# ico-eagleye/OppositeRenderer

Hardware: AMD Instinct MI355X
Metric: Mpaths/s + ms/frame (1080p Sponza PPM) at 1/2/4/8 GPUs; % HBM roofline (higher is better)
Workload: dtype f32

## Files before the change

oppositerenderer_amd/csrc/orx_device.h:

```cpp
#pragma once
#include <hip/hip_runtime.h>
#include <stdint.h>

#include "orx_bvh_nodes.h"
#include "orx_detmath.h"
#include "orx_scene_types.h"

namespace orx {

__host__ __device__ inline bool refract(f3& r, f3 i, f3 n, float ior) {
    f3 nn = n;
    float negNdotV = dot(i, nn);
    float eta;
    if (negNdotV > 0.0f) {
        eta = ior;
        nn = -n;
        negNdotV = -negNdotV;
    } else {
        eta = 1.f / ior;
    }
    const float k = 1.f - eta * eta * (1.f - negNdotV * negNdotV);
    if (k < 0.0f) {
        r = mk1(0.f);
        return false;
    }
    r = normalize(i * eta - nn * (eta * negNdotV + sqrtf(k)));
    return true;
}

constexpr uint32_t PRD_HIT_EMITTER = 1u << 31;
constexpr uint32_t PRD_ERROR = 1u << 30;
constexpr uint32_t PRD_MISS = 1u << 29;
constexpr uint32_t PRD_HIT_SPECULAR = 1u << 28;
constexpr uint32_t PRD_HIT_NON_SPECULAR = 1u << 27;
constexpr uint32_t PRD_PATH_TRACING = 1u << 26;
constexpr float RT_DEFAULT_MAX = 1.e27f;

struct Rng {
    uint32_t v0, v1, v2, v3, v4, d;
};
struct RngPlanes {
    uint32_t* p[6];
};
__device__ __forceinline__ Rng rng_load(const RngPlanes& P, size_t s) {
    return Rng{P.p[0][s], P.p[1][s], P.p[2][s], P.p[3][s], P.p[4][s], P.p[5][s]};
}
__device__ __forceinline__ void rng_store(const RngPlanes& P, size_t s, const Rng& r) {
    P.p[0][s] = r.v0; P.p[1][s] = r.v1; P.p[2][s] = r.v2;
    P.p[3][s] = r.v3; P.p[4][s] = r.v4; P.p[5][s] = r.d;
}
__host__ __device__ __forceinline__ Rng rng_init(uint64_t seed) {
    uint32_t s0 = ((uint32_t)seed) ^ 0xaad26b49u;
    uint32_t s1 = ((uint32_t)(seed >> 32)) ^ 0xf7dcefddu;
    uint32_t t0 = 1099087573u * s0;
    uint32_t t1 = 2591861531u * s1;
    Rng r;
    r.d = 6615241u + t1 + t0;
    r.v0 = 123456789u + t0;
    r.v1 = 362436069u ^ t0;
    r.v2 = 521288629u + t1;
    r.v3 = 88675123u ^ t1;
    r.v4 = 5783321u + t0;
    return r;
}
__host__ __device__ __forceinline__ uint32_t rng_next(Rng& s) {
    uint32_t t = s.v0 ^ (s.v0 >> 2);
    s.v0 = s.v1;
    s.v1 = s.v2;
    s.v2 = s.v3;
    s.v3 = s.v4;
    s.v4 = (s.v4 ^ (s.v4 << 4)) ^ (t ^ (t << 1));
    s.d += 362437u;
    return s.v4 + s.d;
}
__device__ __forceinline__ float rnd(Rng& s) {
    uint32_t x = rng_next(s);
    float u = __builtin_fmaf((float)x, 2.3283064e-10f, 2.3283064e-10f / 2.0f);
    return maxf(u - ORX_FLT_EPSILON, 0.0f);
}

__device__ __forceinline__ void create_coordinate_system(f3 N, f3& U, f3& V) {
    if (fabsf(N.x) > fabsf(N.y)) {
        float invLength = 1.f / sqrtf(N.x * N.x + N.z * N.z);
        U = mk(-N.z * invLength, 0.f, N.x * invLength);
    } else {
        float invLength = 1.f / sqrtf(N.y * N.y + N.z * N.z);
        U = mk(0.f, N.z * invLength, -N.y * invLength);
    }
    V = cross(N, U);
}
__device__ __forceinline__ f3 sample_hemisphere_cos(f3 normal, float sx, float sy) {
    float theta = orx_acosf(sqrtf(sx));
    float phi = 2.0f * ORX_PI_F * sy;
    float st = orx_sinf(theta);
    float xs = st * orx_cosf(phi);
    float ys = orx_cosf(theta);
    float zs = st * orx_sinf(phi);
    f3 U, V;
    create_coordinate_system(normal, U, V);
    return normalize(U * xs + normal * ys + V * zs);
}
__device__ __forceinline__ f3 sample_hemisphere(f3 normal, float sx, float sy) {
    f3 U, V;
    create_coordinate_system(normal, U, V);
    float phi = 2.0f * ORX_PI_F * sx;
    float r = sqrtf(sy);
    float x = r * orx_cosf(phi);
    float y = r * orx_sinf(phi);
    float z = 1.0f - x * x - y * y;
    z = z > 0.0f ? sqrtf(z) : 0.0f;
    return normalize(U * x + V * y + normal * z);
}
__device__ __forceinline__ f3 sample_unit_sphere(float sx, float sy) {
    f3 v;
    v.z = 1.f - 2.f * sx;
    float phi = 2 * ORX_PI_F * sy;
    float r = sqrtf(1.f - v.z * v.z);
    v.x = r * orx_cosf(phi);
    v.y = r * orx_sinf(phi);
    return v;
}
__device__ __forceinline__ f3 sample_disc(float sx, float sy, f3 center, float radius, f3 normal) {
    f3 U, V;
    create_coordinate_system(normal, U, V);
    float r = sqrtf(sx);
    float theta = 2.f * ORX_PI_F * sy;
    float x = r * orx_cosf(theta);
    float y = r * orx_sinf(theta);
    return center + (U * x + V * y) * radius;
}

struct DevScene {
    uint32_t nq, ns, nt;
    const DevQuad* quads;
    const uint32_t* qmat;
    const DevSphere* spheres;
    const uint32_t* smat;
    const float4* tri_v;
    const float4* tri_n;
    const float2* tri_uv;
    const float4* tri_t;
    const float4* tri_bt;
    const DevTexture* tex;
    uint32_t ntex;
    const uint32_t* tmat;
    const DevMaterial* mats;
    const DevLight* lights;
    uint32_t nl;
    float bs_cx, bs_cy, bs_cz, bs_r;
    const DevNode4* bvh4;
    uint32_t bvh_nodes;
    uint32_t stack_entries;
    float dir_zero;
    unsigned long long* trav_stats;
};

#define ORX_STACK_DECL extern __shared__ uint32_t orx_stack_lds[]
#define ORX_STACK_PTR (&orx_stack_lds[threadIdx.x & 63])
#define ORX_STACK_BYTES(S) ((size_t)((S).stack_entries + 2) * 64 * 4)

struct Hit {
    float t;
    int32_t prim;
    uint32_t slot;
    float b, g;
    f3 sn;
};

__device__ __forceinline__ bool isect_quad(const DevQuad& q, f3 o, f3 d, float tmin, float tmax, float& tout) {
    f3 n = mk(q.nx, q.ny, q.nz);
    float dt = dot(d, n);
    float t = (q.d - dot(n, o)) / dt;
    if (t > tmin && t < tmax) {
        f3 p = o + d * t;
        f3 vi = p - mk(q.ax, q.ay, q.az);
        float a1 = dot(mk(q.v1x, q.v1y, q.v1z), vi);
        if (a1 >= 0 && a1 <= 1) {
            float a2 = dot(mk(q.v2x, q.v2y, q.v2z), vi);
            if (a2 >= 0 && a2 <= 1) {
                tout = t;
                return true;
            }
        }
    }
    return false;
}
__device__ __forceinline__ bool isect_sphere(const DevSphere& s, f3 o, f3 d, float tmin, float tmax, float& tout,
                                             f3& nout) {
    f3 O = o - mk(s.cx, s.cy, s.cz);
    float b = dot(O, d);
    float c = dot(O, O) - s.r * s.r;
    float disc = b * b - c;
    if (disc > 0.0f) {
        float sdisc = sqrtf(disc);
        float root1 = (-b - sdisc);
        if (root1 > tmin && root1 < tmax) {
            tout = root1;
            nout = (O + d * root1) / s.r;
            return true;
        }
        float root2 = (-b + sdisc);
        if (root2 > tmin && root2 < tmax) {
            tout = root2;
            nout = (O + d * root2) / s.r;
            return true;
        }
    }
    return false;
}
__device__ __forceinline__ bool isect_tri(f3 p0, f3 p1, f3 p2, f3 o, f3 d, float tmin, float tmax, float& tout,
                                          float& bout, float& gout) {
    f3 e0 = p1 - p0;
    f3 e1 = p0 - p2;
    f3 n = cross(e1, e0);
    f3 e2 = (p0 - o) * (1.0f / dot(n, d));
    f3 i = cross(d, e2);
    float beta = dot(i, e1);
    float gamma = dot(i, e0);
    float t = dot(n, e2);
    if ((t < tmax) & (t > tmin) & (beta >= 0.0f) & (gamma >= 0.0f) & (beta + gamma <= 1)) {
        tout = t;
        bout = beta;
        gout = gamma;
        return true;
    }
    return false;
}
__device__ __forceinline__ f3 ld_f3(const float4& v) { return mk(v.x, v.y, v.z); }

struct RayBox {
    f3 o, inv;
    bool nx, ny, nz;
    f3 oinv;
};
__device__ __forceinline__ RayBox ray_box(f3 o, f3 d, float zero = 1e-30f) {
    auto safe = [zero](float v) { return fabsf(v) > zero ? v : copysignf(zero, v); };
    RayBox rb;
    rb.o = o;
    rb.inv = mk(__builtin_amdgcn_rcpf(safe(d.x)), __builtin_amdgcn_rcpf(safe(d.y)), __builtin_amdgcn_rcpf(safe(d.z)));
    rb.nx = rb.inv.x < 0.f;
    rb.ny = rb.inv.y < 0.f;
    rb.nz = rb.inv.z < 0.f;
    rb.oinv = mk(-o.x * rb.inv.x, -o.y * rb.inv.y, -o.z * rb.inv.z);
    return rb;
}
constexpr float ORX_BOX_TMIN = 1.f - 0x1p-20f, ORX_BOX_TMAX = 1.f + 0x1p-20f;
__device__ __forceinline__ void node_test_q(const float4 A, const float4 B, const float4 C, const float4 D,
                                            const RayBox& rb, float tmin, float tmax, float t[4], uint32_t c[4]) {
    const float sx = A.w, sy = D.z, sz = D.w;
    const float ax = (A.x - rb.o.x) * rb.inv.x, bx = sx * rb.inv.x;
    const float ay = (A.y - rb.o.y) * rb.inv.y, by = sy * rb.inv.y;
    const float az = (A.z - rb.o.z) * rb.inv.z, bz = sz * rb.inv.z;
    const uint32_t lx = __float_as_uint(B.x), ly = __float_as_uint(B.y), lz = __float_as_uint(B.z);
    const uint32_t hx = __float_as_uint(B.w), hy = __float_as_uint(C.x), hz = __float_as_uint(C.y);
    const uint32_t nxq = rb.nx ? hx : lx, fxq = rb.nx ? lx : hx;
    const uint32_t nyq = rb.ny ? hy : ly, fyq = rb.ny ? ly : hy;
    const uint32_t nzq = rb.nz ? hz : lz, fzq = rb.nz ? lz : hz;
    c[0] = __float_as_uint(C.z);
    c[1] = __float_as_uint(C.w);
    c[2] = __float_as_uint(D.x);
    c[3] = __float_as_uint(D.y);
    typedef float v2q __attribute__((ext_vector_type(2)));
    auto q2 = [](uint32_t w, int i) {
        return v2q{(float)((w >> (8 * i)) & 0xffu), (float)((w >> (8 * i + 8)) & 0xffu)};
    };
    const v2q ax2 = v2q{ax, ax}, bx2 = v2q{bx, bx}, ay2 = v2q{ay, ay}, by2 = v2q{by, by};
    const v2q az2 = v2q{az, az}, bz2 = v2q{bz, bz};
#pragma unroll
    for (int h = 0; h < 2; h++) {
        const v2q tnx = __builtin_elementwise_fma(q2(nxq, 2 * h), bx2, ax2);
        const v2q tfx = __builtin_elementwise_fma(q2(fxq, 2 * h), bx2, ax2);
        const v2q tny = __builtin_elementwise_fma(q2(nyq, 2 * h), by2, ay2);
        const v2q tfy = __builtin_elementwise_fma(q2(fyq, 2 * h), by2, ay2);
        const v2q tnz = __builtin_elementwise_fma(q2(nzq, 2 * h), bz2, az2);
        const v2q tfz = __builtin_elementwise_fma(q2(fzq, 2 * h), bz2, az2);
#pragma unroll
        for (int e = 0; e < 2; e++) {
            const int i = 2 * h + e;
            const float t0 = fmaxf(fmaxf(fmaxf(tnx[e], tny[e]), tnz[e]), tmin);
            const float t1 = fminf(fminf(fminf(tfx[e], tfy[e]), tfz[e]), tmax);
            t[i] = t0 <= t1 ? t0 : INFINITY;
        }
    }
}
__device__ __forceinline__ __amdgpu_buffer_rsrc_t orx_rsrc(const void* p) {
    return __builtin_amdgcn_make_buffer_rsrc(const_cast<void*>(p), 0, 0xffffffff, 0x00020000);
}
__device__ __forceinline__ float4 ld16(__amdgpu_buffer_rsrc_t r, uint32_t bo) {
    typedef uint32_t u4b __attribute__((ext_vector_type(4)));
    const u4b v = __builtin_amdgcn_raw_buffer_load_b128(r, (int)bo, 0, 0);
    return make_float4(__uint_as_float(v.x), __uint_as_float(v.y), __uint_as_float(v.z), __uint_as_float(v.w));
}
__device__ __forceinline__ void node_test(const DevBvh4* nodes, uint32_t idx, const RayBox& rb, float tmin, float tmax,
                                          float t[4], uint32_t c[4]) {
    const __amdgpu_buffer_rsrc_t r = orx_rsrc(nodes);
    const uint32_t bo = idx << 6;
    node_test_q(ld16(r, bo), ld16(r, bo + 16), ld16(r, bo + 32), ld16(r, bo + 48), rb, tmin, tmax, t, c);
}
typedef float v2t __attribute__((ext_vector_type(2)));
__device__ __forceinline__ void node_test(const DevBvh4F* nodes, uint32_t idx, const RayBox& rb, float tmin, float tmax,
                                          float t[4], uint32_t c[4]) {
    const float* base = reinterpret_cast<const float*>(nodes + idx);
    const float4 NX = *(const float4*)(base + (rb.nx ? 4 : 0)), FX = *(const float4*)(base + (rb.nx ? 0 : 4));
    const float4 NY = *(const float4*)(base + (rb.ny ? 12 : 8)), FY = *(const float4*)(base + (rb.ny ? 8 : 12));
    const float4 NZ = *(const float4*)(base + (rb.nz ? 20 : 16)), FZ = *(const float4*)(base + (rb.nz ? 16 : 20));
    const uint4 CC = *(const uint4*)(base + 24);
    c[0] = CC.x;
    c[1] = CC.y;
    c[2] = CC.z;
    c[3] = CC.w;
    const v2t ix = v2t{rb.inv.x, rb.inv.x}, iy = v2t{rb.inv.y, rb.inv.y}, iz = v2t{rb.inv.z, rb.inv.z};
    const v2t ox = v2t{rb.oinv.x, rb.oinv.x}, oy = v2t{rb.oinv.y, rb.oinv.y}, oz = v2t{rb.oinv.z, rb.oinv.z};
    const v2t tnx0 = __builtin_elementwise_fma(v2t{NX.x, NX.y}, ix, ox), tnx1 = __builtin_elementwise_fma(v2t{NX.z, NX.w}, ix, ox);
    const v2t tfx0 = __builtin_elementwise_fma(v2t{FX.x, FX.y}, ix, ox), tfx1 = __builtin_elementwise_fma(v2t{FX.z, FX.w}, ix, ox);
    const v2t tny0 = __builtin_elementwise_fma(v2t{NY.x, NY.y}, iy, oy), tny1 = __builtin_elementwise_fma(v2t{NY.z, NY.w}, iy, oy);
    const v2t tfy0 = __builtin_elementwise_fma(v2t{FY.x, FY.y}, iy, oy), tfy1 = __builtin_elementwise_fma(v2t{FY.z, FY.w}, iy, oy);
    const v2t tnz0 = __builtin_elementwise_fma(v2t{NZ.x, NZ.y}, iz, oz), tnz1 = __builtin_elementwise_fma(v2t{NZ.z, NZ.w}, iz, oz);
    const v2t tfz0 = __builtin_elementwise_fma(v2t{FZ.x, FZ.y}, iz, oz), tfz1 = __builtin_elementwise_fma(v2t{FZ.z, FZ.w}, iz, oz);
    const float tn[4][3] = {{tnx0.x, tny0.x, tnz0.x}, {tnx0.y, tny0.y, tnz0.y}, {tnx1.x, tny1.x, tnz1.x}, {tnx1.y, tny1.y, tnz1.y}};
    const float tf[4][3] = {{tfx0.x, tfy0.x, tfz0.x}, {tfx0.y, tfy0.y, tfz0.y}, {tfx1.x, tfy1.x, tfz1.x}, {tfx1.y, tfy1.y, tfz1.y}};
#pragma unroll
    for (int i = 0; i < 4; i++) {
        const float t0 = fmaxf(fmaxf(fmaxf(tn[i][0], tn[i][1]), tn[i][2]), tmin);
        const float t1 = fminf(fminf(fminf(tf[i][0], tf[i][1]), tf[i][2]), tmax);
        t[i] = (t0 <= t1 && c[i] != 0xffffffffu) ? t0 : INFINITY;
    }
}
__device__ __forceinline__ void cswap(float& ta, uint32_t& ca, float& tb, uint32_t& cb) {
    const uint32_t ua = __float_as_uint(ta), ub = __float_as_uint(tb);
    const bool sw = ub < ua;
    const uint32_t c = sw ? cb : ca;
    cb = sw ? ca : cb;
    ca = c;
    ta = __uint_as_float(ua < ub ? ua : ub);
    tb = __uint_as_float(ua < ub ? ub : ua);
}

struct StackL {
    uint32_t* s;
    __device__ __forceinline__ void push(int& sp, uint32_t v) const { s[(sp++) * 64] = v; }
    __device__ __forceinline__ uint32_t pop(int& sp) const { return s[(--sp) * 64]; }
    __device__ __forceinline__ void put(int k, uint32_t v) const { s[k * 64] = v; }
    __device__ __forceinline__ bool shallow(int, int) const { return true; }
    __device__ __forceinline__ void put_l(int k, uint32_t v) const { put(k, v); }
    __device__ __forceinline__ uint32_t pop_l(int& sp) const { return pop(sp); }
};
template <int NL>
struct StackH {
    uint32_t* s;
    __amdgpu_buffer_rsrc_t g;
    uint32_t lane;
    static constexpr uint32_t gstride = 64;
    static constexpr size_t lds_bytes() { return (size_t)(NL + 1) * 64 * 4; }
    __host__ __device__ static constexpr uint32_t deep(uint32_t entries) { return entries + 2 > NL ? entries + 2 - NL : 1u; }
    __device__ __forceinline__ StackH(uint32_t* s_, uint32_t* g_, uint32_t blk, uint32_t ndeep, uint32_t lane_)
        : s(s_), g(__builtin_amdgcn_make_buffer_rsrc(g_ + (size_t)blk * ndeep * 64u, 0, ndeep * 256u, 0x00020000)),
          lane(lane_) {}
    __device__ __forceinline__ void push(int& sp, uint32_t v) const { put(sp++, v); }
    __device__ __forceinline__ uint32_t pop(int& sp) const {
        --sp;
        uint32_t v = s[(sp < NL ? sp : NL) * 64];
        if (sp >= NL) v = __builtin_amdgcn_raw_buffer_load_b32(g, (int)(((uint32_t)(sp - NL) * gstride + lane) * 4u), 0, 0);
        return v;
    }
    __device__ __forceinline__ void put(int k, uint32_t v) const {
        s[(k < NL ? k : NL) * 64] = v;
        if (k >= NL) __builtin_amdgcn_raw_buffer_store_b32(v, g, (int)(((uint32_t)(k - NL) * gstride + lane) * 4u), 0, 0);
    }
    __device__ __forceinline__ bool shallow(int sp, int n) const { return !__ballot(sp + n > NL); }
    __device__ __forceinline__ void put_l(int k, uint32_t v) const { s[k * 64] = v; }
    __device__ __forceinline__ uint32_t pop_l(int& sp) const { return s[(--sp) * 64]; }
};
struct NodesG {
    __device__ __forceinline__ void test(const DevScene& S, uint32_t idx, const RayBox& rb, float tmin, float tmax,
                                         float t[4], uint32_t c[4]) const {
        node_test(S.bvh4, idx, rb, tmin, tmax, t, c);
    }
};

#ifdef ORX_TRAV_STATS
#define ORX_TS_DECL uint32_t ts_nodes = 0, ts_leaves = 0, ts_tris = 0, ts_wn = 0, ts_wl = 0
#define ORX_TS_INC(v, n) (v) += (n)
#define ORX_TS_WAVE(v) (v) += ((uint32_t)(__ffsll((unsigned long long)__ballot(1)) - 1) == (threadIdx.x & 63u))
#define ORX_TS_DECL_TOP uint32_t ts_top[4] = {0, 0, 0, 0}
#define ORX_TS_TOP(idx)                                                     \
    do {                                                                    \
        ts_top[0] += (idx) < 21u;                                           \
        ts_top[1] += (idx) < 85u;                                           \
        ts_top[2] += (idx) < 341u;                                          \
        ts_top[3] += (idx) < 1365u;                                         \
    } while (0)
#define ORX_TS_FLUSH_TOP()                                                  \
    do {                                                                    \
        for (int q_ = 0; q_ < 4; q_++) atomicAdd(&S.trav_stats[16 + q_], (unsigned long long)ts_top[q_]); \
    } while (0)
#define ORX_TS_FLUSH(base)                                                  \
    do {                                                                    \
        atomicAdd(&S.trav_stats[(base) + 0], 1ull);                       \
        atomicAdd(&S.trav_stats[(base) + 1], (unsigned long long)ts_nodes);  \
        atomicAdd(&S.trav_stats[(base) + 2], (unsigned long long)ts_leaves); \
        atomicAdd(&S.trav_stats[(base) + 3], (unsigned long long)ts_tris);   \
        atomicAdd(&S.trav_stats[8 + (base) / 2], (unsigned long long)ts_wn);  \
        atomicAdd(&S.trav_stats[9 + (base) / 2], (unsigned long long)ts_wl);  \
    } while (0)
#else
#define ORX_TS_DECL
#define ORX_TS_DECL_TOP
#define ORX_TS_TOP(idx)
#define ORX_TS_FLUSH_TOP()
#define ORX_TS_INC(v, n)
#define ORX_TS_WAVE(v)
#define ORX_TS_FLUSH(base)
#endif

template <class STK, class NODES>
__device__ inline bool trace_closest_t(const DevScene& S, f3 o, f3 d, float tmin, float tmax, Hit& h, const STK& stk,
                                       const NODES& nodes) {
    float best = tmax;
    int32_t bp = -1;
    uint32_t bslot = 0;
    float t;
    for (uint32_t i = 0; i < S.nq; i++) {
        if (isect_quad(S.quads[i], o, d, tmin, best, t)) {
            best = t;
            bp = (int32_t)i;
        }
    }
    f3 sn = mk1(0);
    for (uint32_t i = 0; i < S.ns; i++) {
        f3 n;
        if (isect_sphere(S.spheres[i], o, d, tmin, best, t, n)) {
            best = t;
            bp = (int32_t)(S.nq + i);
            sn = n;
        }
    }
    float bb = 0, bg = 0;
    if (S.nt) {
        const uint32_t base = S.nq + S.ns;
        const RayBox rb = ray_box(o, d, S.dir_zero);
        const float tmin_box = tmin * ORX_BOX_TMIN;
        int sp = 0;
        uint32_t ref = 0;
        ORX_TS_DECL;
        ORX_TS_DECL_TOP;
        uint32_t lf = 0;
        while (ref != ORX_DONE) {
            while (!(ref & ORX_LEAF) && ref != ORX_DONE) {
                float ct[4];
                uint32_t cc[4];
                nodes.test(S, ref, rb, tmin_box, best * ORX_BOX_TMAX, ct, cc);
                ORX_TS_INC(ts_nodes, 1);
                ORX_TS_TOP(ref);
                ORX_TS_WAVE(ts_wn);
                cswap(ct[0], cc[0], ct[1], cc[1]);
                cswap(ct[2], cc[2], ct[3], cc[3]);
                cswap(ct[0], cc[0], ct[2], cc[2]);
                cswap(ct[1], cc[1], ct[3], cc[3]);
                cswap(ct[1], cc[1], ct[2], cc[2]);
                {
                    const int n3 = ct[3] != INFINITY, n2 = ct[2] != INFINITY, n1 = ct[1] != INFINITY;
                    if (stk.shallow(sp, 3)) {
                        stk.put_l(sp, cc[3]);
                        stk.put_l(sp + n3, cc[2]);
                        stk.put_l(sp + n3 + n2, cc[1]);
                        sp += n3 + n2 + n1;
                        ref = ct[0] != INFINITY ? cc[0] : (sp ? stk.pop_l(sp) : ORX_DONE);
                    } else {
                        stk.put(sp, cc[3]);
                        stk.put(sp + n3, cc[2]);
                        stk.put(sp + n3 + n2, cc[1]);
                        sp += n3 + n2 + n1;
                        ref = ct[0] != INFINITY ? cc[0] : (sp ? stk.pop(sp) : ORX_DONE);
                    }
                }
                if ((ref & ORX_LEAF) && !(lf & ORX_LEAF)) {
                    lf = ref;
                    ref = sp ? stk.pop(sp) : ORX_DONE;
                }
                if (!__ballot(!(lf & ORX_LEAF))) break;
            }
            while (lf & ORX_LEAF) {
                const uint32_t first = (lf & 0x7fffffffu) >> 3, cnt = (lf & 7u) + 1u;
                ORX_TS_INC(ts_leaves, 1);
                ORX_TS_INC(ts_tris, cnt);
                ORX_TS_WAVE(ts_wl);
                const __amdgpu_buffer_rsrc_t tr = orx_rsrc(S.tri_v);
                for (uint32_t k = first; k < first + cnt; k++) {
                    const uint32_t tb = k * 48u;
                    const float4 v0 = ld16(tr, tb), v1 = ld16(tr, tb + 16), v2 = ld16(tr, tb + 32);
                    const int32_t gid = (int32_t)(base + __float_as_uint(v0.w));
                    float b, g;
                    float lim = bp >= 0 ? orx_as_float(orx_as_uint(best) + 1u) : best;
                    if (isect_tri(ld_f3(v0), ld_f3(v1), ld_f3(v2), o, d, tmin, lim, t, b, g) &&
                        (t < best || gid < bp)) {
                        best = t;
                        bp = gid;
                        bslot = k;
                        bb = b;
                        bg = g;
                    }
                }
                lf = ref;
                if (ref & ORX_LEAF) ref = sp ? stk.pop(sp) : ORX_DONE;
            }
        }
        ORX_TS_FLUSH(0);
        ORX_TS_FLUSH_TOP();
    }
    if (bp < 0) return false;
    h.t = best;
    h.prim = bp;
    h.slot = bslot;
    h.b = bb;
    h.g = bg;
    h.sn = sn;
    return true;
}
__device__ __forceinline__ bool trace_closest(const DevScene& S, f3 o, f3 d, float tmin, float tmax, Hit& h,
                                              uint32_t* stk) {
    return trace_closest_t(S, o, d, tmin, tmax, h, StackL{stk}, NodesG{});
}

template <class STK, class NODES>
__device__ inline bool trace_any_t(const DevScene& S, f3 o, f3 d, float tmin, float tmax, const STK& stk,
                                   const NODES& nodes) {
    float t;
    for (uint32_t i = 0; i < S.nq; i++)
        if (isect_quad(S.quads[i], o, d, tmin, tmax, t)) return true;
    for (uint32_t i = 0; i < S.ns; i++) {
        f3 n;
        if (isect_sphere(S.spheres[i], o, d, tmin, tmax, t, n)) return true;
    }
    if (S.nt) {
        const RayBox rb = ray_box(o, d, S.dir_zero);
        const float tmin_box = tmin * ORX_BOX_TMIN, tmax_box = tmax * ORX_BOX_TMAX;
        int sp = 0;
        uint32_t ref = 0;
        ORX_TS_DECL;
        uint32_t lf = 0;
        while (ref != ORX_DONE) {
            while (!(ref & ORX_LEAF) && ref != ORX_DONE) {
                float ct[4];
                uint32_t cc[4];
                nodes.test(S, ref, rb, tmin_box, tmax_box, ct, cc);
                ORX_TS_INC(ts_nodes, 1);
                ORX_TS_WAVE(ts_wn);
                const int h0 = ct[0] != INFINITY, h1 = ct[1] != INFINITY, h2 = ct[2] != INFINITY,
                          h3 = ct[3] != INFINITY;
                const uint32_t next = h3 ? cc[3] : h2 ? cc[2] : h1 ? cc[1] : h0 ? cc[0] : ORX_DONE;
                if (stk.shallow(sp, 4)) {
                    stk.put_l(sp, cc[0]);
                    sp += h0;
                    stk.put_l(sp, cc[1]);
                    sp += h1;
                    stk.put_l(sp, cc[2]);
                    sp += h2;
                    stk.put_l(sp, cc[3]);
                    sp += h3;
                    sp -= next != ORX_DONE;
                    ref = next != ORX_DONE ? next : (sp ? stk.pop_l(sp) : ORX_DONE);
                } else {
                    stk.put(sp, cc[0]);
                    sp += h0;
                    stk.put(sp, cc[1]);
                    sp += h1;
                    stk.put(sp, cc[2]);
                    sp += h2;
                    stk.put(sp, cc[3]);
                    sp += h3;
                    sp -= next != ORX_DONE;
                    ref = next != ORX_DONE ? next : (sp ? stk.pop(sp) : ORX_DONE);
                }
                if ((ref & ORX_LEAF) && !(lf & ORX_LEAF)) {
                    lf = ref;
                    ref = sp ? stk.pop(sp) : ORX_DONE;
                }
                if (!__ballot(!(lf & ORX_LEAF))) break;
            }
            while (lf & ORX_LEAF) {
                const uint32_t first = (lf & 0x7fffffffu) >> 3, cnt = (lf & 7u) + 1u;
                ORX_TS_INC(ts_leaves, 1);
                ORX_TS_WAVE(ts_wl);
                const __amdgpu_buffer_rsrc_t tr = orx_rsrc(S.tri_v);
                for (uint32_t k = first; k < first + cnt; k++) {
                    float b, g;
                    ORX_TS_INC(ts_tris, 1);
                    const uint32_t tb = k * 48u;
                    if (isect_tri(ld_f3(ld16(tr, tb)), ld_f3(ld16(tr, tb + 16)), ld_f3(ld16(tr, tb + 32)), o, d,
                                  tmin, tmax, t, b, g)) {
                        ORX_TS_FLUSH(4);
                        return true;
                    }
                }
                lf = ref;
                if (ref & ORX_LEAF) ref = sp ? stk.pop(sp) : ORX_DONE;
            }
        }
        ORX_TS_FLUSH(4);
    }
    return false;
}

__device__ __forceinline__ bool trace_any(const DevScene& S, f3 o, f3 d, float tmin, float tmax, uint32_t* stk) {
    return trace_any_t(S, o, d, tmin, tmax, StackL{stk}, NodesG{});
}

template <class RAYS, class STK>
__device__ __forceinline__ void trace_any_chain_t(const DevScene& S, RAYS& R, const STK& stk) {
    f3 o = mk1(0.f), d = mk1(0.f);
    float tmin = 0.f, tmax = 0.f, tmin_box = 0.f, tmax_box = 0.f;
    RayBox rb = ray_box(o, mk1(1.f), S.dir_zero);
    int sp = 0;
    uint32_t ref = ORX_DONE, lf = 0;
    auto fetch = [&]() -> bool {
        while (R.next(o, d, tmin, tmax)) {
            float t;
            bool hit = false;
            for (uint32_t i = 0; i < S.nq && !hit; i++) hit = isect_quad(S.quads[i], o, d, tmin, tmax, t);
            for (uint32_t i = 0; i < S.ns && !hit; i++) {
                f3 n;
                hit = isect_sphere(S.spheres[i], o, d, tmin, tmax, t, n);
            }
            if (hit || !S.nt) {
                R.result(hit);
                continue;
            }
            rb = ray_box(o, d, S.dir_zero);
            tmin_box = tmin * ORX_BOX_TMIN, tmax_box = tmax * ORX_BOX_TMAX;
            sp = 0;
            ref = 0;
            lf = 0;
            return true;
        }
        return false;
    };
    bool have = fetch();
    const __amdgpu_buffer_rsrc_t tr = orx_rsrc(S.tri_v);
    while (__ballot(have)) {
        if (!have) continue;
        while (!(ref & ORX_LEAF) && ref != ORX_DONE) {
            float ct[4];
            uint32_t cc[4];
            node_test(S.bvh4, ref, rb, tmin_box, tmax_box, ct, cc);
            const int h0 = ct[0] != INFINITY, h1 = ct[1] != INFINITY, h2 = ct[2] != INFINITY, h3 = ct[3] != INFINITY;
            const uint32_t next = h3 ? cc[3] : h2 ? cc[2] : h1 ? cc[1] : h0 ? cc[0] : ORX_DONE;
            if (stk.shallow(sp, 4)) {
                stk.put_l(sp, cc[0]);
                sp += h0;
                stk.put_l(sp, cc[1]);
                sp += h1;
                stk.put_l(sp, cc[2]);
                sp += h2;
                stk.put_l(sp, cc[3]);
                sp += h3;
                sp -= next != ORX_DONE;
                ref = next != ORX_DONE ? next : (sp ? stk.pop_l(sp) : ORX_DONE);
// ... 527 lines not shown
```

oppositerenderer_amd/csrc/orx_kernels.hip:

```cpp
#include <algorithm>
#include <cstdlib>

#include "orx_kernels.h"

namespace orx {

__device__ __forceinline__ uint32_t f2ord(float f) {
    uint32_t u = __float_as_uint(f);
    return (u & 0x80000000u) ? ~u : (u | 0x80000000u);
}
__device__ __forceinline__ float ord2f(uint32_t u) {
    return __uint_as_float((u & 0x80000000u) ? (u & 0x7fffffffu) : ~u);
}
__device__ __forceinline__ float wave_min(float v) {
    for (int o = 32; o > 0; o >>= 1) v = fminf(v, __shfl_xor(v, o, 64));
    return v;
}
__device__ __forceinline__ float wave_max(float v) {
    for (int o = 32; o > 0; o >>= 1) v = fmaxf(v, __shfl_xor(v, o, 64));
    return v;
}
__device__ __forceinline__ uint64_t wave_sum_u64(uint64_t v) {
    for (int o = 32; o > 0; o >>= 1) v += __shfl_xor(v, o, 64);
    return v;
// ... 163 lines not shown
            M.probe = true;
            M.pdepth = P.depth;
            P.o = hitPoint;
            P.tmin = 0.001f;
            M.tmax = st;
            M.inmed = true;
        }
    } else {
        if (MEDIA) M.tmax = RT_DEFAULT_MAX;
        const DevMaterial& m = S.mats[prim_material(S, h)];
        const f3 hitPoint = P.o + P.d * h.t;
        if (m.type == MAT_DIFFUSE || m.type == MAT_GLOSSY || m.type == MAT_TEXTURE) {
            const bool tex = m.type == MAT_TEXTURE;
            const f3 N = shading_normal(S, h);
            if (P.depth >= 1 && P.numStored < pb.D) {
                const uint32_t si = P.p_local * pb.D + P.numStored;
                float4* rec = pb.slots + 4 * (size_t)si;
                rec[0] = make_float4(hitPoint.x, hitPoint.y, hitPoint.z, P.power.x);
                pb.pos4[si] = make_float4(hitPoint.x, hitPoint.y, hitPoint.z, 0.f);
                rec[1] = make_float4(P.d.x, P.d.y, P.d.z, P.power.y);
                rec[2].x = P.power.z;
                if (fmax3(P.power) > 0 || pb.hash) {
                    P.mask |= 1u << P.numStored;
                    lo_x = fminf(lo_x, hitPoint.x); lo_y = fminf(lo_y, hitPoint.y); lo_z = fminf(lo_z, hitPoint.z);
                    hi_x = fmaxf(hi_x, hitPoint.x); hi_y = fmaxf(hi_y, hitPoint.y); hi_z = fmaxf(hi_z, hitPoint.z);
                }
                P.numStored++;
            }
            const f3 Kd = tex ? tex_color(S, m, h) : m.Kd;
            P.power = P.power * Kd;
            P.weight *= fmax3(Kd);
            if (P.depth >= 3) {
                float probContinue = favgf(Kd);
                float probSample = rnd(rs);
                if (probSample >= probContinue) done = true;
                else P.power = P.power / probContinue;
            }
            if (!done) {
                P.depth++;
                if (P.depth >= c.max_photon_depth || (double)P.weight < (tex ? 0.01 : 0.001) ||
                    P.numStored >= pb.Dlim) {
                    done = true;
                } else {
                    float s0 = rnd(rs);
                    float s1 = rnd(rs);
                    P.d = sample_hemisphere_cos(N, s0, s1);
                    P.o = hitPoint;
                    P.tmin = tex ? 0.01f : 0.0001f;
                    if (MEDIA) M.inmed = false;
                }
            }
        } else if (m.type == MAT_EMITTER) {
            if (MEDIA && !M.inmed) P.depth++;
            done = true;
        } else if (m.type == MAT_MIRROR) {
            const f3 N = shading_normal(S, h);
            P.depth++;
            if (P.depth <= c.max_photon_depth) {
                P.power = P.power * m.Kr;
                P.d = reflect(P.d, N);
                P.o = hitPoint;
                P.tmin = 0.0001f;
                if (MEDIA) M.inmed = false;
            } else {
                done = true;
            }
        } else {
            const f3 wsn = shading_normal(S, h);
            const bool outside = dot(wsn, P.d) < 0;
            const f3 N = outside ? wsn : -wsn;
            const float n1 = outside ? 1.0f : m.ior, n2 = outside ? m.ior : 1.0f;
            f3 refr;
            bool valid;
            const float refl = glass_reflect_factor(P.d, N, n1, n2, refr, valid);
            const float sample = rnd(rs);
            const bool reflected = sample <= refl;
            const f3 nd = reflected ? reflect(P.d, N) : refr;
            P.depth++;
            if (P.depth <= c.max_photon_depth) {
                P.o = hitPoint;
                P.d = nd;
                P.tmin = 0.0001f;
                if (MEDIA) M.inmed = (outside && !reflected) || (!outside && reflected);
            } else {
                done = true;
            }
        }
    }
    if (MEDIA && had_probe && P.depth == M.pdepth) {
        done = true;
        if (rnd(rs) < vm.sig_s / (vm.sig_a + vm.sig_s)) {
            M.nev++;
            M.ev_pos = M.spos;
            M.ev_pow = P.power;
            if (P.depth < c.max_photon_depth) {
                const float s0 = rnd(rs), s1 = rnd(rs);
                P.d = sample_unit_sphere(s0, s1);
                P.o = M.spos;
                P.tmin = 0.001f;
                M.tmax = RT_DEFAULT_MAX;
                M.inmed = false;
                done = false;
            }
        }
    }
    if (done) {
        pb.vmask[P.p_local] = (uint8_t)P.mask;
        rng_store(px.rng, P.slot, rs);
        if (MEDIA) {
            mb.ev_a[P.p_local] = make_float4(M.ev_pos.x, M.ev_pos.y, M.ev_pos.z, __uint_as_float(M.nev));
            mb.ev_b[P.p_local] = make_float4(M.ev_pow.x, M.ev_pow.y, M.ev_pow.z, 0.f);
        }
        return false;
    }
    return true;
}

template <bool MEDIA, class STK, class NODES>
__device__ __forceinline__ bool photon_bounce(const DevScene& S, const PixelBufs& px, const PhotonBufs& pb,
                                              const Consts& c, PhotonPath& P, Rng& rs, const STK& stk,
                                              const NODES& nodes, float& lo_x, float& lo_y, float& lo_z,
                                              float& hi_x, float& hi_y, float& hi_z, const VolMap& vm,
                                              PhotonMedia& M, const MediaBufs& mb) {
    Hit h;
    bool had_probe = false;
    bool hit;
    if (MEDIA) {
        had_probe = M.probe;
        M.probe = false;
        hit = trace_closest_m(S, vm, P.o, P.d, P.tmin, M.tmax, M.inmed, h, stk, nodes);
    } else {
        hit = trace_closest_t(S, P.o, P.d, P.tmin, RT_DEFAULT_MAX, h, stk, nodes);
    }
    return photon_after_hit<MEDIA>(S, px, pb, c, P, rs, hit, h, had_probe, lo_x, lo_y, lo_z, hi_x, hi_y, hi_z, vm, M, mb);
}

__device__ __forceinline__ void photon_bbox_flush(const PhotonBufs& pb, float lo_x, float lo_y, float lo_z, float hi_x,
                                                  float hi_y, float hi_z, uint32_t rep, uint32_t lane) {
    lo_x = wave_min(lo_x); lo_y = wave_min(lo_y); lo_z = wave_min(lo_z);
    hi_x = wave_max(hi_x); hi_y = wave_max(hi_y); hi_z = wave_max(hi_z);
    if (lane < 6) {
        float v = lane == 0 ? lo_x : lane == 1 ? lo_y : lane == 2 ? lo_z : lane == 3 ? hi_x : lane == 4 ? hi_y : hi_z;
        if (lane < 3) {
            if (v != INFINITY) atomicMin(&pb.bbox[lane * BBOX_REPLICAS + rep], f2ord(v));
        } else {
            if (v != -INFINITY) atomicMax(&pb.bbox[lane * BBOX_REPLICAS + rep], f2ord(v));
        }
    }
}

#ifndef ORX_PHOTON_WAVES
#define ORX_PHOTON_WAVES 6
#endif
constexpr int PHOTON_LDS_STACK = 16;
template <bool MEDIA>
__global__ __launch_bounds__(64, ORX_PHOTON_WAVES) void k_ppm_photon(DevScene S, PixelBufs px, PhotonBufs pb, Consts c,
                                                                     MediaBufs mb) {
    ORX_STACK_DECL;
    const uint32_t lane = threadIdx.x;
    const uint32_t total = pb.prows * pb.PW;
    const uint32_t p = blockIdx.x * 64u + lane;
    const StackH<PHOTON_LDS_STACK> stk{ORX_STACK_PTR, pb.tstk, blockIdx.x, pb.tdeep, lane};
    float lo_x = INFINITY, lo_y = INFINITY, lo_z = INFINITY;
    float hi_x = -INFINITY, hi_y = -INFINITY, hi_z = -INFINITY;
    PhotonPath P;
    PhotonMedia M;
    M.tmax = RT_DEFAULT_MAX;
    M.inmed = M.probe = false;
    M.pdepth = M.nev = 0;
    M.spos = M.ev_pos = M.ev_pow = mk1(0.f);
    Rng rs;
    bool alive = p < total;
    if (alive) photon_emit(S, px, pb, p, P, rs);
    while (__ballot(alive)) {
        if (alive)
            alive = photon_bounce<MEDIA>(S, px, pb, c, P, rs, stk, NodesG{}, lo_x, lo_y, lo_z, hi_x, hi_y, hi_z, mb.vm,
                                         M, mb);
    }
    photon_bbox_flush(pb, lo_x, lo_y, lo_z, hi_x, hi_y, hi_z, blockIdx.x & (BBOX_REPLICAS - 1), lane);
}

uint32_t photon_stack_deep(uint32_t entries) { return StackH<PHOTON_LDS_STACK>::deep(entries); }
bool launch_ppm_photon(hipStream_t s, const DevScene& S, const PixelBufs& px, const PhotonBufs& pb, const Consts& c,
                       const MediaBufs* mb) {
    const uint32_t total = pb.prows * pb.PW;
    if (total == 0) return true;
    const uint32_t blocks = (total + 63) / 64;
    if ((size_t)blocks * 64 > pb.tlanes || pb.tdeep < StackH<PHOTON_LDS_STACK>::deep(S.stack_entries)) return false;
    const size_t lds = StackH<PHOTON_LDS_STACK>::lds_bytes();
    if (mb)
        hipLaunchKernelGGL((k_ppm_photon<true>), dim3(blocks), dim3(64), lds, s, S, px, pb, c, *mb);
    else
        hipLaunchKernelGGL((k_ppm_photon<false>), dim3(blocks), dim3(64), lds, s, S, px, pb, c, MediaBufs{});
    return true;
}

__global__ void k_grid_setup(PhotonBufs pb, GridBox gb) {
    __shared__ uint32_t red[6];
    const uint32_t lane = threadIdx.x;
    for (int k = 0; k < 6; k++) {
        uint32_t v = pb.bbox[k * BBOX_REPLICAS + lane];
        for (int o = 32; o > 0; o >>= 1) {
            uint32_t w = (uint32_t)__shfl_xor((int)v, o, 64);
            v = k < 3 ? min(v, w) : max(v, w);
        }
        if (lane == 0) red[k] = v;
        pb.bbox[k * BBOX_REPLICAS + lane] = k < 3 ? 0xffffffffu : 0u;
    }
    __syncthreads();
    if (lane != 0) return;
    uint32_t b[6];
    GridParams* g = pb.grid;
    const bool own = red[0] != 0xffffffffu;
    for (int k = 0; k < 3; k++) {
        g->clo[k] = own ? ord2f(red[k]) : INFINITY;
        g->chi[k] = own ? ord2f(red[k + 3]) : -INFINITY;
    }
    for (int k = 0; k < 6; k++) b[k] = gb.on ? gb.b[k] : red[k];
    bool any = b[0] != 0xffffffffu;
    f3 lo, hi;
    if (any) {
        lo = mk(ord2f(b[0]), ord2f(b[1]), ord2f(b[2]));
        hi = mk(ord2f(b[3]), ord2f(b[4]), ord2f(b[5]));
    } else {
        lo = mk1(0.f);
        hi = mk1(0.f);
    }
    lo = mk(lo.x - 0.0000001f, lo.y - 0.0000001f, lo.z - 0.0000001f);
    hi = mk(hi.x + 0.0000001f, hi.y + 0.0000001f, hi.z + 0.0000001f);
    f3 ext = hi - lo;
    float sceneVolume = ext.x * ext.y * ext.z;
    float minVolumePerCell = sceneVolume / (float)pb.gcells;
    float radiusC = orx_powf(minVolumePerCell, 1.0f / 3.0f);
    f3 ncf = ext / radiusC;
    uint32_t nx = orx_f2u_sat(orx_floorf(ncf.x)), ny = orx_f2u_sat(orx_floorf(ncf.y)),
             nz = orx_f2u_sat(orx_floorf(ncf.z));
    f3 each = mk(ext.x / (float)nx, ext.y / (float)ny, ext.z / (float)nz);
    float smallest = fmax3(each);
    float cellSize = (float)((double)smallest + 0.001);
    f3 f = ext / cellSize;
    uint32_t gx = orx_f2u_sat(orx_ceilf(f.x)), gy = orx_f2u_sat(orx_ceilf(f.y)), gz = orx_f2u_sat(orx_ceilf(f.z));
    gx = gx < 1 ? 1 : gx;
    gy = gy < 1 ? 1 : gy;
    gz = gz < 1 ? 1 : gz;
    uint64_t G = (uint64_t)gx * gy * gz;
    g->ox = lo.x; g->oy = lo.y; g->oz = lo.z;
    g->cell = cellSize;
    g->gx = gx; g->gy = gy; g->gz = gz;
    g->any_valid = any;
    g->photons_visited = 0;
    g->cells_visited = 0;
    if (G > pb.gmax) {
        g->error = 1;
        g->G = 0;
    } else {
        g->error = 0;
        g->G = (uint32_t)G;
    }
}
void launch_grid_setup(hipStream_t s, const PhotonBufs& pb, const GridBox& gb) {
    hipLaunchKernelGGL(k_grid_setup, dim3(1), dim3(64), 0, s, pb, gb);
}

constexpr int SCAN_BLOCK = 1024;

__device__ __forceinline__ uint32_t block_exclusive_scan_256(uint32_t v, uint32_t* total) {
    __shared__ uint32_t ws[4];
    const int lane = threadIdx.x & 63, w = threadIdx.x >> 6;
    uint32_t x = v;
    for (int o = 1; o < 64; o <<= 1) {
        uint32_t y = __shfl_up(x, o, 64);
        if (lane >= o) x += y;
    }
    if (lane == 63) ws[w] = x;
    __syncthreads();
    uint32_t pre = 0;
    for (int q = 0; q < w; q++) pre += ws[q];
    *total = ws[0] + ws[1] + ws[2] + ws[3];
    __syncthreads();
    return pre + x - v;
}

constexpr int32_t DIRQ_BAND = 232;
__device__ __forceinline__ uint32_t dir_q8(float x, float y, float z) {
    if (!(fabsf(x) + fabsf(y) + fabsf(z) <= 1.7325f) || !(fmaxf(fabsf(x), fmaxf(fabsf(y), fabsf(z))) <= 1.0f))
        return 0u;
    const int32_t qx = (int32_t)rintf(x * 127.f), qy = (int32_t)rintf(y * 127.f), qz = (int32_t)rintf(z * 127.f);
    return ((uint32_t)qx & 0xffu) | (((uint32_t)qy & 0xffu) << 8) | (((uint32_t)qz & 0xffu) << 16);
}

__device__ __forceinline__ void grid_put(const PhotonBufs& pb, uint32_t dst, const float4 a, const float4 b, float cz) {
    const size_t P = pb.splane;
    float* o = pb.sorted + dst;
    o[SP_X * P] = a.x;
    o[SP_Y * P] = a.y;
    o[SP_Z * P] = a.z;
    o[SP_DIRQ * P] = __uint_as_float(dir_q8(b.x, b.y, b.z));
    o[SP_DX * P] = b.x;
    o[SP_DY * P] = b.y;
    o[SP_DZ * P] = b.z;
    o[SP_PX * P] = a.w;
    o[SP_PY * P] = b.w;
    o[SP_PZ * P] = cz;
}
__global__ __launch_bounds__(256) void k_grid_permute(PhotonBufs pb) {
    const uint32_t valid = pb.grid->valid;
    const uint32_t T = gridDim.x * blockDim.x;
// ... 1420 lines not shown
```

Before: 1101.

## Use LDS byte-address stack pointer with sentinel and branchless push offsets

Rewrites the BVH traversal stack in trace_closest to track a raw LDS byte address instead of an integer index. An ORX_DONE sentinel sits at the stack base so pops need no empty check. Push offsets come from boolean hit masks instead of comparisons against INFINITY. A separate deep path handles spilling to the global buffer, and the LDS stack grows by one entry to hold the sentinel. The aim is fewer address computations and branches per node visit, at the cost of more code and slightly more LDS per wave, which could reduce occupancy.

```diff
diff --git a/oppositerenderer_amd/csrc/orx_device.h b/oppositerenderer_amd/csrc/orx_device.h
--- a/oppositerenderer_amd/csrc/orx_device.h
+++ b/oppositerenderer_amd/csrc/orx_device.h
@@ -157,7 +157,12 @@
 
 #define ORX_STACK_DECL extern __shared__ uint32_t orx_stack_lds[]
 #define ORX_STACK_PTR (&orx_stack_lds[threadIdx.x & 63])
-#define ORX_STACK_BYTES(S) ((size_t)((S).stack_entries + 2) * 64 * 4)
+#define ORX_STACK_BYTES(S) ((size_t)((S).stack_entries + 3) * 64 * 4)
+typedef __attribute__((address_space(3))) uint32_t orx_lds_u32;
+constexpr uint32_t ORX_STK_STRIDE = 64 * 4;
+__device__ __forceinline__ uint32_t orx_lds_addr(uint32_t* p) { return (uint32_t)(uintptr_t)(orx_lds_u32*)p; }
+__device__ __forceinline__ void orx_lds_st(uint32_t a, uint32_t v) { *(orx_lds_u32*)(uintptr_t)a = v; }
+__device__ __forceinline__ uint32_t orx_lds_ld(uint32_t a) { return *(orx_lds_u32*)(uintptr_t)a; }
 
 struct Hit {
     float t;
@@ -246,7 +251,8 @@
 }
 constexpr float ORX_BOX_TMIN = 1.f - 0x1p-20f, ORX_BOX_TMAX = 1.f + 0x1p-20f;
 __device__ __forceinline__ void node_test_q(const float4 A, const float4 B, const float4 C, const float4 D,
-                                            const RayBox& rb, float tmin, float tmax, float t[4], uint32_t c[4]) {
+                                            const RayBox& rb, float tmin, float tmax, float t[4], uint32_t c[4],
+                                            bool* hit = nullptr, const float miss = INFINITY) {
     const float sx = A.w, sy = D.z, sz = D.w;
     const float ax = (A.x - rb.o.x) * rb.inv.x, bx = sx * rb.inv.x;
     const float ay = (A.y - rb.o.y) * rb.inv.y, by = sy * rb.inv.y;
@@ -279,7 +285,8 @@
             const int i = 2 * h + e;
             const float t0 = fmaxf(fmaxf(fmaxf(tnx[e], tny[e]), tnz[e]), tmin);
             const float t1 = fminf(fminf(fminf(tfx[e], tfy[e]), tfz[e]), tmax);
-            t[i] = t0 <= t1 ? t0 : INFINITY;
+            t[i] = t0 <= t1 ? t0 : miss;
+            if (hit) hit[i] = t0 <= t1;
         }
     }
 }
@@ -292,14 +299,14 @@
     return make_float4(__uint_as_float(v.x), __uint_as_float(v.y), __uint_as_float(v.z), __uint_as_float(v.w));
 }
 __device__ __forceinline__ void node_test(const DevBvh4* nodes, uint32_t idx, const RayBox& rb, float tmin, float tmax,
-                                          float t[4], uint32_t c[4]) {
+                                          float t[4], uint32_t c[4], bool* hit = nullptr, const float miss = INFINITY) {
     const __amdgpu_buffer_rsrc_t r = orx_rsrc(nodes);
     const uint32_t bo = idx << 6;
-    node_test_q(ld16(r, bo), ld16(r, bo + 16), ld16(r, bo + 32), ld16(r, bo + 48), rb, tmin, tmax, t, c);
+    node_test_q(ld16(r, bo), ld16(r, bo + 16), ld16(r, bo + 32), ld16(r, bo + 48), rb, tmin, tmax, t, c, hit, miss);
 }
 typedef float v2t __attribute__((ext_vector_type(2)));
 __device__ __forceinline__ void node_test(const DevBvh4F* nodes, uint32_t idx, const RayBox& rb, float tmin, float tmax,
-                                          float t[4], uint32_t c[4]) {
+                                          float t[4], uint32_t c[4], bool* hit = nullptr, const float miss = INFINITY) {
     const float* base = reinterpret_cast<const float*>(nodes + idx);
     const float4 NX = *(const float4*)(base + (rb.nx ? 4 : 0)), FX = *(const float4*)(base + (rb.nx ? 0 : 4));
     const float4 NY = *(const float4*)(base + (rb.ny ? 12 : 8)), FY = *(const float4*)(base + (rb.ny ? 8 : 12));
@@ -323,7 +330,9 @@
     for (int i = 0; i < 4; i++) {
         const float t0 = fmaxf(fmaxf(fmaxf(tn[i][0], tn[i][1]), tn[i][2]), tmin);
         const float t1 = fminf(fminf(fminf(tf[i][0], tf[i][1]), tf[i][2]), tmax);
-        t[i] = (t0 <= t1 && c[i] != 0xffffffffu) ? t0 : INFINITY;
+        const bool hi = t0 <= t1 && c[i] != 0xffffffffu;
+        t[i] = hi ? t0 : miss;
+        if (hit) hit[i] = hi;
     }
 }
 __device__ __forceinline__ void cswap(float& ta, uint32_t& ca, float& tb, uint32_t& cb) {
@@ -344,6 +353,14 @@
     __device__ __forceinline__ bool shallow(int, int) const { return true; }
     __device__ __forceinline__ void put_l(int k, uint32_t v) const { put(k, v); }
     __device__ __forceinline__ uint32_t pop_l(int& sp) const { return pop(sp); }
+    __device__ __forceinline__ uint32_t addr0() const { return orx_lds_addr(s); }
+    __device__ __forceinline__ bool shallow_a(uint32_t, int, bool) const { return true; }
+    __device__ __forceinline__ void put_a(uint32_t a, uint32_t off, uint32_t v) const { orx_lds_st(a + off, v); }
+    __device__ __forceinline__ uint32_t pop_a(uint32_t& a) const {
+        const uint32_t v = orx_lds_ld(a);
+        a -= ORX_STK_STRIDE;
+        return v;
+    }
 };
 template <int NL>
 struct StackH {
@@ -352,7 +369,7 @@
     uint32_t lane;
     static constexpr uint32_t gstride = 64;
     static constexpr size_t lds_bytes() { return (size_t)(NL + 1) * 64 * 4; }
-    __host__ __device__ static constexpr uint32_t deep(uint32_t entries) { return entries + 2 > NL ? entries + 2 - NL : 1u; }
+    __host__ __device__ static constexpr uint32_t deep(uint32_t entries) { return entries + 3 > NL ? entries + 3 - NL : 1u; }
     __device__ __forceinline__ StackH(uint32_t* s_, uint32_t* g_, uint32_t blk, uint32_t ndeep, uint32_t lane_)
         : s(s_), g(__builtin_amdgcn_make_buffer_rsrc(g_ + (size_t)blk * ndeep * 64u, 0, ndeep * 256u, 0x00020000)),
           lane(lane_) {}
@@ -370,11 +387,27 @@
     __device__ __forceinline__ bool shallow(int sp, int n) const { return !__ballot(sp + n > NL); }
     __device__ __forceinline__ void put_l(int k, uint32_t v) const { s[k * 64] = v; }
     __device__ __forceinline__ uint32_t pop_l(int& sp) const { return s[(--sp) * 64]; }
+    __device__ __forceinline__ uint32_t addr0() const { return orx_lds_addr(s); }
+    __device__ __forceinline__ uint32_t lim() const { return orx_lds_addr(s - lane) + (uint32_t)NL * ORX_STK_STRIDE; }
+    __device__ __forceinline__ bool shallow_a(uint32_t a, int n, bool need) const {
+        return !__ballot(need && a >= lim() - (uint32_t)n * ORX_STK_STRIDE);
+    }
+    __device__ __forceinline__ void put_a(uint32_t a, uint32_t off, uint32_t v) const {
+        if (a >= lim() - off) __builtin_amdgcn_raw_buffer_store_b32(v, g, (int)(a - (lim() - off)), 0, 0);
+        else orx_lds_st(a + off, v);
+    }
+    __device__ __forceinline__ uint32_t pop_a(uint32_t& a) const {
+        uint32_t v;
+        if (a >= lim()) v = __builtin_amdgcn_raw_buffer_load_b32(g, (int)(a - lim()), 0, 0);
+        else v = orx_lds_ld(a);
+        a -= ORX_STK_STRIDE;
+        return v;
+    }
 };
 struct NodesG {
     __device__ __forceinline__ void test(const DevScene& S, uint32_t idx, const RayBox& rb, float tmin, float tmax,
-                                         float t[4], uint32_t c[4]) const {
-        node_test(S.bvh4, idx, rb, tmin, tmax, t, c);
+                                         float t[4], uint32_t c[4], bool* hit = nullptr, const float miss = INFINITY) const {
+        node_test(S.bvh4, idx, rb, tmin, tmax, t, c, hit, miss);
     }
 };
 
@@ -440,45 +473,72 @@
         const uint32_t base = S.nq + S.ns;
         const RayBox rb = ray_box(o, d, S.dir_zero);
         const float tmin_box = tmin * ORX_BOX_TMIN;
-        int sp = 0;
+        const uint32_t a0 = stk.addr0();
+        orx_lds_st(a0, ORX_DONE);
+        uint32_t a = a0;
         uint32_t ref = 0;
         ORX_TS_DECL;
         ORX_TS_DECL_TOP;
         uint32_t lf = 0;
+        auto front = [&](uint32_t cc[4], uint32_t& n1, uint32_t& n2, uint32_t& n3, bool& h1) {
+            float ct[4];
+            bool m[4];
+            nodes.test(S, ref, rb, tmin_box, best * ORX_BOX_TMAX, ct, cc, m, __uint_as_float(0xffffffffu));
+            ORX_TS_INC(ts_nodes, 1);
+            ORX_TS_TOP(ref);
+            ORX_TS_WAVE(ts_wn);
+            cswap(ct[0], cc[0], ct[1], cc[1]);
+            cswap(ct[2], cc[2], ct[3], cc[3]);
+            cswap(ct[0], cc[0], ct[2], cc[2]);
+            cswap(ct[1], cc[1], ct[3], cc[3]);
+            cswap(ct[1], cc[1], ct[2], cc[2]);
+            const bool mp = m[0] && m[1], mq = m[2] && m[3], mr = m[0] || m[1], ms = m[2] || m[3];
+            const bool h2 = mp || mq || (mr && ms), h3 = (mp && ms) || (mq && mr), h4 = mp && mq;
+            h1 = mr || ms;
+            n3 = h4 ? ORX_STK_STRIDE : 0u, n2 = h3 ? ORX_STK_STRIDE : 0u, n1 = h2 ? ORX_STK_STRIDE : 0u;
+        };
         while (ref != ORX_DONE) {
+            bool deep = false;
             while (!(ref & ORX_LEAF) && ref != ORX_DONE) {
-                float ct[4];
-                uint32_t cc[4];
-                nodes.test(S, ref, rb, tmin_box, best * ORX_BOX_TMAX, ct, cc);
-                ORX_TS_INC(ts_nodes, 1);
-                ORX_TS_TOP(ref);
-                ORX_TS_WAVE(ts_wn);
-                cswap(ct[0], cc[0], ct[1], cc[1]);
-                cswap(ct[2], cc[2], ct[3], cc[3]);
-                cswap(ct[0], cc[0], ct[2], cc[2]);
-                cswap(ct[1], cc[1], ct[3], cc[3]);
-                cswap(ct[1], cc[1], ct[2], cc[2]);
-                {
-                    const int n3 = ct[3] != INFINITY, n2 = ct[2] != INFINITY, n1 = ct[1] != INFINITY;
-                    if (stk.shallow(sp, 3)) {
-                        stk.put_l(sp, cc[3]);
-                        stk.put_l(sp + n3, cc[2]);
-                        stk.put_l(sp + n3 + n2, cc[1]);
-                        sp += n3 + n2 + n1;
-                        ref = ct[0] != INFINITY ? cc[0] : (sp ? stk.pop_l(sp) : ORX_DONE);
-                    } else {
-                        stk.put(sp, cc[3]);
-                        stk.put(sp + n3, cc[2]);
-                        stk.put(sp + n3 + n2, cc[1]);
-                        sp += n3 + n2 + n1;
-                        ref = ct[0] != INFINITY ? cc[0] : (sp ? stk.pop(sp) : ORX_DONE);
-                    }
+                if (!stk.shallow_a(a, 3, true)) {
+                    deep = true;
+                    break;
+                }
+                uint32_t cc[4], n1, n2, n3;
+                bool h1;
+                front(cc, n1, n2, n3, h1);
+                const uint32_t a1 = a + n3, a2 = a1 + n2;
+                orx_lds_st(a + ORX_STK_STRIDE, cc[3]);
+                orx_lds_st(a1 + ORX_STK_STRIDE, cc[2]);
+                orx_lds_st(a2 + ORX_STK_STRIDE, cc[1]);
+                a = a2 + n1;
+                ref = cc[0];
+                if (!h1) {
+                    ref = orx_lds_ld(a);
+                    a -= ORX_STK_STRIDE;
                 }
                 if ((ref & ORX_LEAF) && !(lf & ORX_LEAF)) {
                     lf = ref;
-                    ref = sp ? stk.pop(sp) : ORX_DONE;
+                    ref = orx_lds_ld(a);
+                    a -= ORX_STK_STRIDE;
                 }
                 if (!__ballot(!(lf & ORX_LEAF))) break;
+            }
+            if (deep && !(ref & ORX_LEAF) && ref != ORX_DONE) {
+                uint32_t cc[4], n1, n2, n3;
+                bool h1;
+                front(cc, n1, n2, n3, h1);
+                const uint32_t a1 = a + n3, a2 = a1 + n2;
+                stk.put_a(a, ORX_STK_STRIDE, cc[3]);
+                stk.put_a(a1, ORX_STK_STRIDE, cc[2]);
+                stk.put_a(a2, ORX_STK_STRIDE, cc[1]);
+                a = a2 + n1;
+                ref = cc[0];
+                if (!h1) ref = stk.pop_a(a);
+                if ((ref & ORX_LEAF) && !(lf & ORX_LEAF)) {
+                    lf = ref;
+                    ref = stk.pop_a(a);
+                }
             }
             while (lf & ORX_LEAF) {
                 const uint32_t first = (lf & 0x7fffffffu) >> 3, cnt = (lf & 7u) + 1u;
@@ -502,7 +562,14 @@
                     }
                 }
                 lf = ref;
-                if (ref & ORX_LEAF) ref = sp ? stk.pop(sp) : ORX_DONE;
+                if (stk.shallow_a(a, 0, ref & ORX_LEAF)) {
+                    if (ref & ORX_LEAF) {
+                        ref = orx_lds_ld(a);
+                        a -= ORX_STK_STRIDE;
+                    }
+                } else if (ref & ORX_LEAF) {
+                    ref = stk.pop_a(a);
+                }
             }
         }
         ORX_TS_FLUSH(0);
diff --git a/oppositerenderer_amd/csrc/orx_kernels.hip b/oppositerenderer_amd/csrc/orx_kernels.hip
--- a/oppositerenderer_amd/csrc/orx_kernels.hip
+++ b/oppositerenderer_amd/csrc/orx_kernels.hip
@@ -339,7 +339,7 @@
 #ifndef ORX_PHOTON_WAVES
 #define ORX_PHOTON_WAVES 6
 #endif
-constexpr int PHOTON_LDS_STACK = 16;
+constexpr int PHOTON_LDS_STACK = 17;
 template <bool MEDIA>
 __global__ __launch_bounds__(64, ORX_PHOTON_WAVES) void k_ppm_photon(DevScene S, PixelBufs px, PhotonBufs pb, Consts c,
                                                                      MediaBufs mb) {
```

Result: no change. 1110 (median of 6 runs) (+0.9%).
